# minh86/ModelCrowdNav

Hardware: AMD Instinct MI355X
Metric: env-steps/sec (whole node), 5-human CrowdSim x batched envs (higher is better)
Workload: dtype f64

## Files before the change

modelcrowdnav_amd/csrc/env_rollout_quad.hip:

```cpp
#include <hip/hip_runtime.h>
#include <stdint.h>
#include "../../include/mcn.h"
#include "quad_common.hpp"
#include "env_step_params.hpp"
#include "env_common.hpp"

namespace mcn {
void note_dispatch(const char *family);
void note_rollout_form(int form);

#ifdef MCN_DIAG
#define MCN_STAMP_SLOTS 64
#define MCN_STAMP_WAVES 8192
__device__ unsigned long long g_stamps[MCN_STAMP_WAVES * MCN_STAMP_SLOTS];
#define STAMP(slot)                                                                                              \
    do {                                                                                                         \
        const int w_ = blockIdx.x * (blockDim.x >> 6) + (threadIdx.x >> 6);                                      \
        if ((threadIdx.x & 63) == 0 && (slot) < MCN_STAMP_SLOTS && w_ < MCN_STAMP_WAVES)                         \
            g_stamps[w_ * MCN_STAMP_SLOTS + (slot)] = __builtin_amdgcn_s_memrealtime();                          \
    } while (0)
#define STAMP_WHERE()                                                                                            \
    do {                                                                                                         \
        const int w_ = blockIdx.x * (blockDim.x >> 6) + (threadIdx.x >> 6);                                      \
        if ((threadIdx.x & 63) == 0 && w_ < MCN_STAMP_WAVES)                                                     \
            g_stamps[w_ * MCN_STAMP_SLOTS + 38] =                                                                \
                (unsigned long long)__builtin_amdgcn_s_getreg((4) | (0 << 6) | (31 << 11)) |                     \
                ((unsigned long long)__builtin_amdgcn_s_getreg((20) | (0 << 6) | (31 << 11)) << 32);             \
    } while (0)
int read_counts(void *dst, size_t bytes, int reset)
{
    if (bytes > sizeof(g_diag_counts)) bytes = sizeof(g_diag_counts);
    const int rc = hipMemcpyFromSymbol(dst, HIP_SYMBOL(g_diag_counts), bytes) == hipSuccess ? (int)(bytes / 4) : -1;
    if (reset) {
        void *sym = nullptr;
        if (hipGetSymbolAddress(&sym, HIP_SYMBOL(g_diag_counts)) == hipSuccess) (void)hipMemset(sym, 0, sizeof(g_diag_counts));
    }
    return rc;
}
int read_stamps(void *dst, size_t bytes)
{
    if (bytes > sizeof(g_stamps)) bytes = sizeof(g_stamps);
    return hipMemcpyFromSymbol(dst, HIP_SYMBOL(g_stamps), bytes) == hipSuccess ? (int)(bytes / 8) : -1;
}
#else
#define STAMP(slot)
#define STAMP_WHERE()
#endif

__device__ __forceinline__ int bperm_i(int byte_addr, int v) { return __builtin_amdgcn_ds_bpermute(byte_addr, v); }
__device__ __forceinline__ float bperm_f(int byte_addr, float v)
{
    return __builtin_bit_cast(float, bperm_i(byte_addr, __builtin_bit_cast(int, v)));
}
__device__ __forceinline__ double bperm_d(int byte_addr, double v)
{
    const long long b = __builtin_bit_cast(long long, v);
    const int lo = bperm_i(byte_addr, (int)b), hi = bperm_i(byte_addr, (int)(b >> 32));
    return __builtin_bit_cast(double, ((long long)hi << 32) | (unsigned int)lo);
}

template <class V>
__device__ __forceinline__ V in_vgpr(V v)
{
    asm volatile("" : "+v"(v));
    return v;
}

typedef const __attribute__((address_space(4))) StepParams *KernargPtr;
__device__ __forceinline__ KernargPtr kernarg_here()
{
    KernargPtr q = (KernargPtr)__builtin_amdgcn_kernarg_segment_ptr();
    asm volatile("" : "+s"(q));
    return q;
}

template <int NT>
struct Wg4 {
    static_assert(NT == 5, "the four-wavefront form is built for 5 humans only");
    static constexpr int EW = 8;
    static constexpr int NQ = EW * NT;
};

template <int CTRL>
__device__ __forceinline__ int dpp_i(int v) { return __builtin_amdgcn_mov_dpp(v, CTRL, 0xf, 0xf, true); }
template <int CTRL>
__device__ __forceinline__ double dpp_d(double v)
{
    const long long b = __builtin_bit_cast(long long, v);
    const int lo = dpp_i<CTRL>((int)b), hi = dpp_i<CTRL>((int)(b >> 32));
    return __builtin_bit_cast(double, ((long long)hi << 32) | (unsigned int)lo);
}
constexpr int DPP_QUAD_XOR1 = 0xB1, DPP_QUAD_XOR2 = 0x4E, DPP_ROW_HALF_MIRROR = 0x141;

template <int NT, int VIS, bool UNI>
__device__ __forceinline__ void rollout_wg4(const StepParams &p, const int T)
{
    static_assert(VIS == 0, "the four-wavefront form is built for an invisible robot only");
    constexpr int EW = Wg4<NT>::EW, NQ = Wg4<NT>::NQ;
    __shared__ float4 s_opa[NQ], s_opb[NQ];
    __shared__ float2 s_res[NQ];
    __shared__ double2 s_hpos[NQ];
    __shared__ double s_hrad[NQ];
    STAMP(0);
    STAMP_WHERE();
#ifdef MCN_DIAG
    if (p.debug_noop) return;
#endif
    const int tid = threadIdx.x;
    const int role = __builtin_amdgcn_readfirstlane(tid >> 6);
    const unsigned nb_ = gridDim.x, xcd_ = blockIdx.x & 7u, idx_ = blockIdx.x >> 3;
    const unsigned qq_ = nb_ >> 3, rr__ = nb_ & 7u;
    const unsigned chunk_ = (xcd_ < rr__ ? xcd_ * (qq_ + 1) : rr__ * (qq_ + 1) + (xcd_ - rr__) * qq_) + idx_;
    const mcn_env_cfg &c = p.cfg;
    const mcn_rollout &ro = p.roll;

    if (role < 3) {
        const int lane = tid & 63, k = tid & 3, q = tid >> 2;
        const bool pop = q < NQ;
        const int ge = q / NT, h = q - ge * NT;
        const bool active = pop && (long)chunk_ * EW + ge < p.E;
        const int hi = pop ? q : 0;
        const bool cand_h = k < NT - 1;
        const int j = cand_h ? k + (k >= h ? 1 : 0) : h;
        const int ci = pop ? ge * NT + j : 0;
        const bool publish = pop && k == 0;
        const float inv_th = in_vgpr(1.0f / c.orca_time_horizon), inv_ts = in_vgpr(1.0f / (float)c.time_step);
        __syncthreads();
        STAMP(1);

        for (int t = 0; t < T; ++t) {
            const float4 A = s_opa[hi], B = s_opb[hi], o = s_opa[ci];
            const float orad = s_opb[ci].z;
            float rx, ry;
            quad_orca_core(c, lane, k, cand_h && active, A, B, o, orad, inv_th, inv_ts, rx, ry);
            if (publish) s_res[hi] = make_float2(rx, ry);
            if (t < 20) STAMP(40 + t);
            __syncthreads();
            __syncthreads();
            if (t < 37) STAMP(2 + t);
        }
    } else {
        static_assert(EW * 8 == 64, "eight lanes per env fill the wavefront");
        const double dt = in_vgpr(c.time_step);
        const bool do_reset = p.has_roll && ro.pool_hpos != nullptr;
        const int l = tid & 63;
        const int g = l >> 3, h = l & 7;
        const bool pop = h < NT;
        const int hs = g * NT + (pop ? h : 0);
        const long e = (long)chunk_ * EW + g;
        const bool active = pop && e < p.E;
        const long eb = e < p.E ? e : 0;
        const long a = eb * NT + (pop ? h : 0);
        const bool lead = active && h == 0;
        constexpr bool unicycle = UNI;
        const bool has_state = p.has_roll && ro.state != nullptr;
        const bool track = c.track_human_times && p.st.human_times != nullptr;

        double2 pos = reinterpret_cast<const double2 *>(p.st.hpos)[a];
        double2 vel = reinterpret_cast<const double2 *>(p.st.hvel)[a];
        double2 goal = reinterpret_cast<const double2 *>(p.st.hgoal)[a];
        double rad = p.st.hrad[a];
        double vpref = p.st.hvpref[a];
        double htime = p.st.human_times ? p.st.human_times[a] : 0.0;
        double hax = 0, hay = 0;
        double2 rpos = reinterpret_cast<const double2 *>(p.st.rpos)[eb];
        double2 rvel = reinterpret_cast<const double2 *>(p.st.rvel)[eb];
        double2 rgoal = reinterpret_cast<const double2 *>(p.st.rgoal)[eb];
        const double rrad = p.st.rrad[eb];
        double gtime = p.st.gtime[eb];
        double rtheta = p.st.rtheta ? p.st.rtheta[eb] : 0.0;
        mcn_roll_rec rs = {0, 0, 0, 0, 0, 0};
        if (has_state) rs = ro.state[eb];
        const double2 *act_ptr = reinterpret_cast<const double2 *>(p.actions) + eb;
        const long act_stride = in_vgpr((long)p.E);
        const double *disc_table = in_vgpr(ro.disc_table);
        const int disc_last = in_vgpr(ro.disc_len - 1);
        const bool has_theta = p.st.rtheta != nullptr;
        double2 act_next = *act_ptr;
        double o_rew = 0, o_dmin = 0;
        int o_dn = 0, o_inf = 0, o_hh = 0;
        const double k_timeout_at = in_vgpr(c.time_limit - 1);
        const double k_collision = in_vgpr(c.collision_penalty), k_success = in_vgpr(c.success_reward);
        const double k_discomfort = in_vgpr(c.discomfort_dist), k_factor = in_vgpr(c.discomfort_penalty_factor);
        const int k_stride = ro.case_stride, k_pool = ro.pool_size;
        const bool count_hh = c.count_hh != 0;
        {
            float4 A, B;
            quad_orca_operands(c, pos, vel, goal, rad, vpref, A, B);
            if (pop) { s_opa[hs] = A; s_opb[hs] = B; s_hpos[hs] = pos; s_hrad[hs] = rad; }
        }
        __syncthreads();
        STAMP(1);

        for (int t = 0; t < T; ++t) {
            const double2 act = act_next;
            act_ptr += act_stride;
            if (t + 1 < T) act_next = *act_ptr;
            double ep_disc = 0;
            if (has_state) ep_disc = disc_table[rs.ep_steps < disc_last ? rs.ep_steps : disc_last];

            double2 eff = act;
            if (unicycle) {
                eff.x = act.x * cos(act.y + rtheta);
                eff.y = act.x * sin(act.y + rtheta);
            }
            double cd;
            {
                const double px = pos.x - rpos.x, py = pos.y - rpos.y;
                const double vx = vel.x - eff.x, vy = vel.y - eff.y;
                cd = p2s_origin(px, py, px + vx * dt, py + vy * dt) - rad - rrad;
            }
            cd = pop ? cd : INFINITY;
            int hh = 0;
            {
                static_assert(NT / 2 == 2, "two pairs per lane");
                double s2[2], ra[2], rb[2];
                bool near_any = false;
                const bool counted = active & count_hh;
#pragma unroll
                for (int d = 1; d <= NT / 2; ++d) {
                    const int jj = h + d >= NT ? h + d - NT : h + d;
                    const int pi = g * NT + (pop ? jj : 0);
                    const double2 ppos = s_hpos[pi];
                    const double prad = s_hrad[pi];
                    ra[d - 1] = jj > h ? rad : prad; rb[d - 1] = jj > h ? prad : rad;
                    const double dx = pos.x - ppos.x, dy = pos.y - ppos.y;
                    s2[d - 1] = dx * dx + dy * dy;
                    const double reach = ra[d - 1] + rb[d - 1] + 1e-6;
                    near_any |= counted & (s2[d - 1] < reach * reach);
                }
                if (__any(near_any)) {
                    DIAG_COUNT(2);
#pragma unroll
                    for (int d = 0; d < NT / 2; ++d)
                        hh += (counted & ((sqrt(s2[d]) - ra[d] - rb[d]) < 0)) ? 1 : 0;
                }
            }
            double dmin = cd;
            int hh_sum = hh;
            dmin = fmin(dmin, dpp_d<DPP_QUAD_XOR1>(dmin));       hh_sum += dpp_i<DPP_QUAD_XOR1>(hh_sum);
            dmin = fmin(dmin, dpp_d<DPP_QUAD_XOR2>(dmin));       hh_sum += dpp_i<DPP_QUAD_XOR2>(hh_sum);
            dmin = fmin(dmin, dpp_d<DPP_ROW_HALF_MIRROR>(dmin)); hh_sum += dpp_i<DPP_ROW_HALF_MIRROR>(hh_sum);

            double endx, endy, new_theta = rtheta, nrvx, nrvy;
            if (unicycle) {
                const double th = rtheta + act.y;
                endx = rpos.x + cos(th) * act.x * dt;
                endy = rpos.y + sin(th) * act.x * dt;
                new_theta = pymod(rtheta + act.y, 2 * M_PI);
                nrvx = act.x * cos(new_theta); nrvy = act.x * sin(new_theta);
            } else {
                endx = rpos.x + act.x * dt; endy = rpos.y + act.y * dt;
                nrvx = act.x; nrvy = act.y;
            }
            bool reaching = false;
            {
                const double gx = endx - rgoal.x, gy = endy - rgoal.y, near = rrad + 1e-6;
                if (__any(gx * gx + gy * gy < near * near)) DIAG_COUNT(3);
                if (__any(gx * gx + gy * gy < near * near)) reaching = norm2(gx, gy) < rrad;
            }
            double rew; int inf, dn;
            if (gtime >= k_timeout_at)          { rew = 0; dn = 1; inf = MCN_INFO_TIMEOUT; }
            else if (dmin < 0)                  { rew = k_collision; dn = 1; inf = MCN_INFO_COLLISION; }
            else if (reaching)                  { rew = k_success; dn = 1; inf = MCN_INFO_REACHGOAL; }
            else if (dmin < k_discomfort)       { rew = (dmin - k_discomfort) * k_factor * dt; dn = 0; inf = MCN_INFO_DANGER; }
            else                                { rew = 0; dn = 0; inf = MCN_INFO_NOTHING; }
            o_rew = rew; o_dmin = dmin; o_dn = dn; o_inf = inf; o_hh = hh_sum;
            const double t_new = gtime + dt;

            const int case_g = rs.next_case;
            if (has_state) {
                bool danger = inf == MCN_INFO_DANGER;
                if (danger) {
                    const KernargPtr kp = kernarg_here();
                    const int lim = kp->roll.danger_episodes, sf = kp->roll.danger_short_from;
                    danger = lim <= 0 || rs.fin_count < lim - ((sf > 0 && e >= sf - 1) ? 1 : 0);
                }
                rs.danger_count += danger ? 1 : 0;
                rs.danger_dist_sum = danger ? rs.danger_dist_sum + dmin : rs.danger_dist_sum;
                const double ret = rs.ep_return + ep_disc * rew;
                if (lead && dn) {
                    const int kf = rs.fin_count;
                    const KernargPtr kp = kernarg_here();
                    const int fin_slots = kp->roll.fin_slots;
                    double *fin_return = kp->roll.fin_return, *fin_time = kp->roll.fin_time;
                    uint8_t *fin_info = kp->roll.fin_info;
                    const bool keep = (fin_slots == 1) || (kf < fin_slots);
                    const long rec = (long)(fin_slots == 1 ? 0 : kf) * kp->E + e;
                    if (keep && fin_return) fin_return[rec] = ret;
                    if (keep && fin_time)   fin_time[rec] = (inf == MCN_INFO_TIMEOUT) ? kp->cfg.time_limit : t_new;
                    if (keep && fin_info)   fin_info[rec] = (uint8_t)inf;
                }
                rs.fin_count += dn;
                rs.ep_return = dn ? 0.0 : ret;
                rs.ep_steps = dn ? 0 : rs.ep_steps + 1;
                if (do_reset) {
                    int nc = rs.next_case + k_stride;
                    nc = nc >= k_pool ? nc - k_pool : nc;
                    rs.next_case = dn ? nc : rs.next_case;
                }
            }

            if (do_reset && dn) {
                const KernargPtr kp = kernarg_here();
                const double k_theta0 = kp->roll.robot_theta0;
                rpos = make_double2(kp->roll.robot_start[0], kp->roll.robot_start[1]);
                rgoal = make_double2(kp->roll.robot_goal[0], kp->roll.robot_goal[1]);
                rvel = make_double2(0, 0);
                if (has_theta) rtheta = k_theta0;
                gtime = 0;
            } else {
                rpos = make_double2(endx, endy);
                rvel = make_double2(nrvx, nrvy);
                if (unicycle) rtheta = new_theta;
                gtime = t_new;
            }

            double2 npos = pos, nvel = vel, ngoal = goal;
            double nrad = rad, nvpref = vpref;
            if (do_reset && dn) {
                DIAG_COUNT(1);
                if (active) {
                    const long pa = (long)case_g * NT + h;
                    const KernargPtr kp = kernarg_here();
                    const double2 *pool_hvel = reinterpret_cast<const double2 *>(kp->roll.pool_hvel);
                    nvel = make_double2(0, 0);
                    if (pool_hvel) nvel = pool_hvel[pa];
                    npos = reinterpret_cast<const double2 *>(kp->roll.pool_hpos)[pa];
                    ngoal = reinterpret_cast<const double2 *>(kp->roll.pool_hgoal)[pa];
                    nrad = kp->roll.pool_hrad[pa];
                    nvpref = kp->roll.pool_hvpref[pa];
                }
            }

            if (t < 20) STAMP(40 + t);
            __syncthreads();
            {
                const float2 r = s_res[hs];
                hax = (double)r.x; hay = (double)r.y;
            }

            if (do_reset && dn) {
                pos = npos; vel = nvel; goal = ngoal; rad = nrad; vpref = nvpref;
                htime = 0;
            } else {
                pos = make_double2(pos.x + hax * dt, pos.y + hay * dt);
                vel = make_double2(hax, hay);
                if (track && htime == 0 && norm2(pos.x - goal.x, pos.y - goal.y) < rad) htime = t_new;
            }
            {
                float4 A, B;
                quad_orca_operands(c, pos, vel, goal, rad, vpref, A, B);
                if (pop) { s_opa[hs] = A; s_opb[hs] = B; s_hpos[hs] = pos; s_hrad[hs] = rad; }
            }
            __syncthreads();
            if (t < 37) STAMP(2 + t);
        }

        long a2 = a, e2 = e;
        asm volatile("" : "+v"(a2), "+v"(e2));
        const KernargPtr kp = kernarg_here();
        if (active) {
            reinterpret_cast<double2 *>(kp->st.hpos)[a2] = pos;
            reinterpret_cast<double2 *>(kp->st.hvel)[a2] = vel;
            if (do_reset) {
                reinterpret_cast<double2 *>(kp->st.hgoal)[a2] = goal;
                kp->st.hrad[a2] = rad;
                kp->st.hvpref[a2] = vpref;
            }
            double *human_times = kp->st.human_times, *human_act = kp->out.human_act;
            if (human_times) human_times[a2] = htime;
            if (human_act) reinterpret_cast<double2 *>(human_act)[a2] = make_double2(hax, hay);
        }
        if (lead) {
            reinterpret_cast<double2 *>(kp->st.rpos)[e2] = rpos;
            reinterpret_cast<double2 *>(kp->st.rvel)[e2] = rvel;
            if (do_reset) reinterpret_cast<double2 *>(kp->st.rgoal)[e2] = rgoal;
            double *rth = kp->st.rtheta;
            if (rth) rth[e2] = rtheta;
            kp->st.gtime[e2] = gtime;
            store_step_rec(kp->out.rec + e2, o_rew, o_dmin, o_dn, o_inf, o_hh);
            if (has_state) kp->roll.state[e2] = rs;
        }
    }
    STAMP(39);
}

template <int NT, int VIS, bool UNI>
__global__ __launch_bounds__(256, 2) void env_rollout_wg4_kernel(const StepParams p, const int T)
{
    rollout_wg4<NT, VIS, UNI>(p, T);
}

template <int NT, int VIS, bool UNI, bool SPLIT>
__global__ __launch_bounds__(SPLIT ? 128 : 64, SPLIT ? 3 : 1) void env_rollout_quad_kernel(const StepParams p, const int T)
{
    __shared__ double2 s_hpos[16], s_hvel[16], s_rpos[16], s_rvel[16];
    __shared__ double s_hrad[16];
    __shared__ int s_dn[16], s_case[16];
    STAMP(0);
    STAMP_WHERE();
#ifdef MCN_DIAG
    if (p.debug_noop) return;
#endif
    const int role = SPLIT ? (int)(threadIdx.x >> 6) : -1;
    const bool do_orca = role != 1, do_pair = role != 0;
    constexpr int NC = NT - 1 + VIS;
    constexpr int LPE = 4 * NT;
    constexpr int G = 64 / LPE;
    static_assert(NC >= 0 && NC <= 4, "quad kernel handles at most 4 ORCA neighbours");
    const int lane = threadIdx.x & 63;
    const int g = lane / LPE;
    const int r = lane - g * LPE;
    const int h = r >> 2, k = r & 3;
#ifndef MCN_QUAD_XCD
#define MCN_QUAD_XCD 1
#endif
    const unsigned nb_ = gridDim.x, xcd_ = blockIdx.x & 7u, idx_ = blockIdx.x >> 3;
    const unsigned qq_ = nb_ >> 3, rr__ = nb_ & 7u;
    const unsigned chunk_ = MCN_QUAD_XCD ? (xcd_ < rr__ ? xcd_ * (qq_ + 1) : rr__ * (qq_ + 1) + (xcd_ - rr__) * qq_) + idx_
                                         : blockIdx.x;
    const long e = (long)chunk_ * G + g;
    const bool active = (g < G) && (e < p.E);
    const long eb = active ? e : 0;
    const long a = eb * NT + h;
    const int gi = g < G ? g : 0;
    const int hi = g < G ? g * NT + h : 0;
    const mcn_env_cfg &c = p.cfg;
    const mcn_rollout &ro = p.roll;
    const double dt = in_vgpr(c.time_step);
    const bool lead = active && r == 0 && do_pair;
    const bool hlead = active && k == 0 && do_orca;
    constexpr bool unicycle = UNI;
    const bool has_state = p.has_roll && ro.state != nullptr;
    const bool do_reset = p.has_roll && ro.pool_hpos != nullptr;
    const bool track = c.track_human_times && p.st.human_times != nullptr;

    double2 pos = reinterpret_cast<const double2 *>(p.st.hpos)[a];
    double2 vel = reinterpret_cast<const double2 *>(p.st.hvel)[a];
    double2 goal = reinterpret_cast<const double2 *>(p.st.hgoal)[a];
    double rad = p.st.hrad[a];
    double vpref = p.st.hvpref[a];
    double htime = p.st.human_times ? p.st.human_times[a] : 0.0;
    double2 rpos = reinterpret_cast<const double2 *>(p.st.rpos)[eb];
    double2 rvel = reinterpret_cast<const double2 *>(p.st.rvel)[eb];
    double2 rgoal = reinterpret_cast<const double2 *>(p.st.rgoal)[eb];
    const double rrad = p.st.rrad[eb];
    double gtime = p.st.gtime[eb];
    double rtheta = p.st.rtheta ? p.st.rtheta[eb] : 0.0;
    mcn_roll_rec rs = {0, 0, 0, 0, 0, 0};
    if (has_state) rs = ro.state[eb];

    const bool cand_h = k < NT - 1;
    const bool cand_r = VIS && (k == NT - 1);
    const int j = cand_h ? k + (k >= h ? 1 : 0) : h;
    const int l0 = lane - r;
    const int src = ((l0 + 4 * j) & 63) << 2;

    const double2 *act_ptr = reinterpret_cast<const double2 *>(p.actions) + eb;
    const long act_stride = in_vgpr((long)p.E);
    const double *disc_table = in_vgpr(ro.disc_table);
    const int disc_last = in_vgpr(ro.disc_len - 1);
    const bool has_theta = p.st.rtheta != nullptr;
    double2 act_next = *act_ptr;
    double o_rew = 0, o_dmin = 0;
    int o_dn = 0, o_inf = 0, o_hh = 0;
    double hax = 0, hay = 0;
    const float inv_th = in_vgpr(1.0f / c.orca_time_horizon), inv_ts = in_vgpr(1.0f / (float)c.time_step);
    STAMP(1);

    for (int t = 0; t < T; ++t) {
        const double2 act = act_next;
        act_ptr += act_stride;
        if (do_pair && t + 1 < T) act_next = *act_ptr;
        double ep_disc = 0;
        if (do_pair && has_state) ep_disc = disc_table[rs.ep_steps < disc_last ? rs.ep_steps : disc_last];

        double2 cpos;
        cpos.x = bperm_d(src, pos.x);
        cpos.y = bperm_d(src, pos.y);
        double crd = bperm_d(src, rad);
        float cvx = bperm_f(src, (float)vel.x), cvy = bperm_f(src, (float)vel.y);
        if (cand_r) { cpos = rpos; crd = rrad; }

        int dn = 0, case_g = 0;
        double t_new = 0;

        if (do_orca) {
            if (cand_r) { cvx = (float)rvel.x; cvy = (float)rvel.y; }
            float rx, ry;
            quad_orca_velocity(c, lane, k, (cand_h || cand_r) && active, pos, vel, goal, rad, vpref,
                               make_float4((float)cpos.x, (float)cpos.y, cvx, cvy), crd, inv_th, inv_ts, rx, ry);
            hax = (double)rx; hay = (double)ry;
        }

        if (do_pair) {
            double2 eff = act;
            if (unicycle) {
                eff.x = act.x * cos(act.y + rtheta);
                eff.y = act.x * sin(act.y + rtheta);
            }
            double cd;
            {
                const double px = pos.x - rpos.x, py = pos.y - rpos.y;
                const double vx = vel.x - eff.x, vy = vel.y - eff.y;
                cd = p2s_origin(px, py, px + vx * dt, py + vy * dt) - rad - rrad;
            }
            int hh = 0;
            {
                const double dx = pos.x - cpos.x, dy = pos.y - cpos.y;
                const bool counted = active & (c.count_hh != 0) & cand_h & (j > h);
                const double s2 = dx * dx + dy * dy, reach = rad + crd + 1e-6;
                if (__any(counted & (s2 < reach * reach))) DIAG_COUNT(2);
                if (__any(counted & (s2 < reach * reach)))
                    hh = (counted & ((sqrt(s2) - rad - crd) < 0)) ? 1 : 0;
            }
            hh += __builtin_amdgcn_update_dpp(0, hh, 0xB1, 0xf, 0xf, false);
            hh += __builtin_amdgcn_update_dpp(0, hh, 0x4E, 0xf, 0xf, false);
            double dmin = INFINITY;
            int hh_sum = 0;
#pragma unroll
            for (int q = 0; q < NT; ++q) {
                const int s = (l0 + 4 * q) & 63;
                dmin = fmin(dmin, __shfl(cd, s));
                hh_sum += __shfl(hh, s);
            }

            double endx, endy, new_theta = rtheta, nrvx, nrvy;
            if (unicycle) {
                const double th = rtheta + act.y;
                endx = rpos.x + cos(th) * act.x * dt;
                endy = rpos.y + sin(th) * act.x * dt;
                new_theta = pymod(rtheta + act.y, 2 * M_PI);
                nrvx = act.x * cos(new_theta); nrvy = act.x * sin(new_theta);
            } else {
                endx = rpos.x + act.x * dt; endy = rpos.y + act.y * dt;
                nrvx = act.x; nrvy = act.y;
            }
            bool reaching = false;
            {
                const double gx = endx - rgoal.x, gy = endy - rgoal.y, near = rrad + 1e-6;
                if (__any(gx * gx + gy * gy < near * near)) DIAG_COUNT(3);
                if (__any(gx * gx + gy * gy < near * near)) reaching = norm2(gx, gy) < rrad;
            }
            const KernargPtr kc = kernarg_here();
            const double k_time_limit = kc->cfg.time_limit, k_timeout_at = k_time_limit - 1;
            const double k_collision = kc->cfg.collision_penalty, k_success = kc->cfg.success_reward;
            const double k_discomfort = kc->cfg.discomfort_dist, k_factor = kc->cfg.discomfort_penalty_factor;
            double rew; int inf;
            if (gtime >= k_timeout_at)          { rew = 0; dn = 1; inf = MCN_INFO_TIMEOUT; }
            else if (dmin < 0)                  { rew = k_collision; dn = 1; inf = MCN_INFO_COLLISION; }
            else if (reaching)                  { rew = k_success; dn = 1; inf = MCN_INFO_REACHGOAL; }
            else if (dmin < k_discomfort)       { rew = (dmin - k_discomfort) * k_factor * dt; dn = 0; inf = MCN_INFO_DANGER; }
            else                                { rew = 0; dn = 0; inf = MCN_INFO_NOTHING; }
            o_rew = rew; o_dmin = dmin; o_dn = dn; o_inf = inf; o_hh = hh_sum;
            t_new = gtime + dt;

            case_g = rs.next_case;
            if (has_state) {
                bool danger = inf == MCN_INFO_DANGER;
                if (danger) {
                    const KernargPtr kp = kernarg_here();
                    const int lim = kp->roll.danger_episodes, sf = kp->roll.danger_short_from;
                    danger = lim <= 0 || rs.fin_count < lim - ((sf > 0 && e >= sf - 1) ? 1 : 0);
                }
                rs.danger_count += danger ? 1 : 0;
                rs.danger_dist_sum = danger ? rs.danger_dist_sum + dmin : rs.danger_dist_sum;
                const double ret = rs.ep_return + ep_disc * rew;
                if (lead && dn) {
                    const int kf = rs.fin_count;
                    const KernargPtr kp = kernarg_here();
                    const int fin_slots = kp->roll.fin_slots;
                    double *fin_return = kp->roll.fin_return, *fin_time = kp->roll.fin_time;
                    uint8_t *fin_info = kp->roll.fin_info;
                    const bool keep = (fin_slots == 1) || (kf < fin_slots);
                    const long rec = (long)(fin_slots == 1 ? 0 : kf) * kp->E + e;
                    if (keep && fin_return) fin_return[rec] = ret;
                    if (keep && fin_time)   fin_time[rec] = (inf == MCN_INFO_TIMEOUT) ? k_time_limit : t_new;
                    if (keep && fin_info)   fin_info[rec] = (uint8_t)inf;
                }
                rs.fin_count += dn;
                rs.ep_return = dn ? 0.0 : ret;
                rs.ep_steps = dn ? 0 : rs.ep_steps + 1;
                if (do_reset) {
                    const int k_stride = kc->roll.case_stride, k_pool = kc->roll.pool_size;
                    int nc = rs.next_case + k_stride;
                    nc = nc >= k_pool ? nc - k_pool : nc;
                    rs.next_case = dn ? nc : rs.next_case;
                }
            }

            if (do_reset && dn) {
                const KernargPtr kp = kernarg_here();
                const double k_theta0 = kp->roll.robot_theta0;
                rpos = make_double2(kp->roll.robot_start[0], kp->roll.robot_start[1]);
                rgoal = make_double2(kp->roll.robot_goal[0], kp->roll.robot_goal[1]);
                rvel = make_double2(0, 0);
                if (has_theta) rtheta = k_theta0;
                gtime = 0;
            } else {
                rpos = make_double2(endx, endy);
                rvel = make_double2(nrvx, nrvy);
                if (unicycle) rtheta = new_theta;
                gtime = t_new;
            }
        }

        if (SPLIT) {
            if (lead) {
                s_dn[gi] = dn; s_case[gi] = case_g;
                if (VIS) { s_rpos[gi] = rpos; s_rvel[gi] = rvel; }
            }
            __syncthreads();
            if (role == 0) {
                dn = s_dn[gi]; case_g = s_case[gi];
                if (VIS) { rpos = s_rpos[gi]; rvel = s_rvel[gi]; }
            }
        }

        if (do_orca) {
            if (do_reset && dn) {
                DIAG_COUNT(1);
                if (active) {
                    const long pa = (long)case_g * NT + h;
                    const KernargPtr kp = kernarg_here();
                    const double2 *pool_hvel = reinterpret_cast<const double2 *>(kp->roll.pool_hvel);
                    pos = reinterpret_cast<const double2 *>(kp->roll.pool_hpos)[pa];
                    goal = reinterpret_cast<const double2 *>(kp->roll.pool_hgoal)[pa];
                    rad = kp->roll.pool_hrad[pa];
                    vpref = kp->roll.pool_hvpref[pa];
                    vel = pool_hvel ? pool_hvel[pa] : make_double2(0, 0);
                }
                htime = 0;
            } else {
                pos = make_double2(pos.x + hax * dt, pos.y + hay * dt);
                vel = make_double2(hax, hay);
                if (track && htime == 0 && norm2(pos.x - goal.x, pos.y - goal.y) < rad) htime = SPLIT ? gtime + dt : t_new;
            }
        }
        if (SPLIT) {
            if (role == 0) gtime = (do_reset && dn) ? 0.0 : gtime + dt;
            if (hlead) { s_hpos[hi] = pos; s_hvel[hi] = vel; s_hrad[hi] = rad; }
            __syncthreads();
            if (role == 1) { pos = s_hpos[hi]; vel = s_hvel[hi]; rad = s_hrad[hi]; }
        }
        if (t < 37) STAMP(2 + t);
    }

    {
        long a2 = a, e2 = e;
        asm volatile("" : "+v"(a2), "+v"(e2));
        const KernargPtr kp = kernarg_here();
        if (hlead) {
            reinterpret_cast<double2 *>(kp->st.hpos)[a2] = pos;
            reinterpret_cast<double2 *>(kp->st.hvel)[a2] = vel;
            if (do_reset) {
                reinterpret_cast<double2 *>(kp->st.hgoal)[a2] = goal;
                kp->st.hrad[a2] = rad;
                kp->st.hvpref[a2] = vpref;
            }
            double *human_times = kp->st.human_times, *human_act = kp->out.human_act;
            if (human_times) human_times[a2] = htime;
            if (human_act) reinterpret_cast<double2 *>(human_act)[a2] = make_double2(hax, hay);
        }
        if (lead) {
            reinterpret_cast<double2 *>(kp->st.rpos)[e2] = rpos;
            reinterpret_cast<double2 *>(kp->st.rvel)[e2] = rvel;
            if (do_reset) reinterpret_cast<double2 *>(kp->st.rgoal)[e2] = rgoal;
            double *rth = kp->st.rtheta;
            if (rth) rth[e2] = rtheta;
            kp->st.gtime[e2] = gtime;
            store_step_rec(kp->out.rec + e2, o_rew, o_dmin, o_dn, o_inf, o_hh);
            if (has_state) kp->roll.state[e2] = rs;
        }
    }
    STAMP(39);
}

template <int NT, int VIS, bool UNI>
static void launch_rollout_kin(const StepParams &p, int T, int blocks, hipStream_t stream)
{
    if constexpr (NT == 5 && VIS == 0) {
        if (p.quad_split == 2) {
            constexpr int EW = Wg4<NT>::EW;
            hipLaunchKernelGGL((env_rollout_wg4_kernel<NT, VIS, UNI>), dim3((p.E + EW - 1) / EW), dim3(256), 0, stream, p, T);
            note_rollout_form(2);
            return;
        }
    }
    if (p.quad_split)
        hipLaunchKernelGGL((env_rollout_quad_kernel<NT, VIS, UNI, true>), dim3(blocks), dim3(128), 0, stream, p, T);
    else
        hipLaunchKernelGGL((env_rollout_quad_kernel<NT, VIS, UNI, false>), dim3(blocks), dim3(64), 0, stream, p, T);
    note_rollout_form(p.quad_split ? 1 : 0);
}

template <int NT, int VIS>
static void launch_rollout_one(const StepParams &p, int T, hipStream_t stream)
{
    constexpr int G = 64 / (4 * NT);
    const int blocks = (p.E + G - 1) / G;
    if (p.cfg.robot_kinematics == MCN_KIN_UNICYCLE)
        launch_rollout_kin<NT, VIS, true>(p, T, blocks, stream);
    else
        launch_rollout_kin<NT, VIS, false>(p, T, blocks, stream);
}

bool launch_env_rollout_quad(const StepParams &p, int T, hipStream_t stream)
{
    if (p.cfg.human_policy != MCN_HUMANS_ORCA || p.cfg.orca_max_neighbors < 4 || !p.update) return false;
    const int vis = p.cfg.robot_visible ? 1 : 0;
    const int nc = p.N - 1 + vis;
    if (nc > 4 || p.N < 1) return false;
    switch (p.N * 2 + vis) {
        case 2:  launch_rollout_one<1, 0>(p, T, stream); break;
        case 3:  launch_rollout_one<1, 1>(p, T, stream); break;
        case 4:  launch_rollout_one<2, 0>(p, T, stream); break;
        case 5:  launch_rollout_one<2, 1>(p, T, stream); break;
        case 6:  launch_rollout_one<3, 0>(p, T, stream); break;
        case 7:  launch_rollout_one<3, 1>(p, T, stream); break;
        case 8:  launch_rollout_one<4, 0>(p, T, stream); break;
        case 9:  launch_rollout_one<4, 1>(p, T, stream); break;
        case 10: launch_rollout_one<5, 0>(p, T, stream); break;
        default: return false;
    }
    note_dispatch("env_rollout_quad_kernel");
    return true;
}

}
```

modelcrowdnav_amd/csrc/quad_common.hpp:

```cpp
#pragma once
#include <hip/hip_runtime.h>
#include "orca_device.hpp"
#include "orca_static.hpp"

namespace mcn {

#ifdef MCN_DIAG
static __device__ unsigned int g_diag_counts[8192 * 4];
#define DIAG_COUNT(which)                                                                                        \
    do {                                                                                                         \
        const int w_ = blockIdx.x * (blockDim.x >> 6) + (threadIdx.x >> 6);                                      \
        if (w_ < 8192 && (int)(threadIdx.x & 63) == __ffsll((unsigned long long)__ballot(1)) - 1)                \
            atomicAdd(&g_diag_counts[w_ * 4 + (which)], 1u);                                                     \
    } while (0)
#else
#define DIAG_COUNT(which)
#endif

template <int I>
__device__ __forceinline__ int qbi(int v) { return __builtin_amdgcn_mov_dpp(v, I * 0x55, 0xf, 0xf, false); }
template <int I>
__device__ __forceinline__ float qbf(float v) { return __builtin_bit_cast(float, qbi<I>(__builtin_bit_cast(int, v))); }
template <int I>
__device__ __forceinline__ double qbd(double v)
{
    const long long b = __builtin_bit_cast(long long, v);
    const int lo = qbi<I>((int)b), hi = qbi<I>((int)(b >> 32));
    return __builtin_bit_cast(double, ((long long)hi << 32) | (unsigned int)lo);
}
template <int I>
__device__ __forceinline__ float4 qb4(float4 v) { return make_float4(qbf<I>(v.x), qbf<I>(v.y), qbf<I>(v.z), qbf<I>(v.w)); }

__device__ __forceinline__ float4 sel4(const float4 (&L)[4], int i)
{
    const float4 a = i == 1 ? L[1] : L[0], b = i == 3 ? L[3] : L[2];
    return i >= 2 ? b : a;
}

template <bool DIR>
__device__ __forceinline__ bool lp1_rt(const float4 (&L)[4], const float4 &ln, int no, float radius, float optx, float opty,
                                       float &rx, float &ry)
{
    const float dp = dot2(ln.x, ln.y, ln.z, ln.w);
    const float disc = dp * dp + radius * radius - dot2(ln.x, ln.y, ln.x, ln.y);
    bool ok = !(disc < 0.0f);
    const float sq = sqrt_f32(disc, ok);
    float tl = -dp - sq;
    float tr = -dp + sq;
#pragma unroll
    for (int i = 0; i < 3; ++i) {
        const float4 li = L[i];
        const float den = det2(ln.z, ln.w, li.z, li.w);
        const float num = det2(li.z, li.w, ln.x - li.x, ln.y - li.y);
        const float t = num / den;
        const bool live = i < no;
        const bool par = fabsf(den) <= kRvoEps;
        const bool cut = live & !par;
        const float ntr = fminf(tr, t), ntl = fmaxf(tl, t);
        tr = (cut & (den >= 0.0f)) ? ntr : tr;
        tl = (cut & !(den >= 0.0f)) ? ntl : tl;
        ok = ok & !(live & ((par ? 0.0f : tl) > (par ? num : tr)));
    }
    float t;
    if (DIR) {
        t = (dot2(optx, opty, ln.z, ln.w) > 0.0f) ? tr : tl;
    } else {
        t = dot2(ln.z, ln.w, optx - ln.x, opty - ln.y);
        if (t < tl) t = tl; else if (t > tr) t = tr;
    }
    rx = ln.x + t * ln.z;
    ry = ln.y + t * ln.w;
    return ok;
}

__device__ __forceinline__ bool lp3_candidate_quad(const float4 &li, const float4 &lj, int i, int k, float radius, float &rx,
                                                   float &ry)
{
    const float dt = det2(li.z, li.w, lj.z, lj.w);
    const bool par = fabsf(dt) <= kRvoEps;
    const bool same = dot2(li.z, li.w, lj.z, lj.w) > 0.0f;
    const bool keptb = (k < i) & !(par & same);
    const unsigned long long m_kept = lanes(k < i) & ~(lanes(par) & lanes(same));
    const float sc = det2(lj.z, lj.w, li.x - lj.x, li.y - lj.y) / dt;
    const float ddx = lj.z - li.z, ddy = lj.w - li.w;
    const float inv = keptb ? rcp_sqrt_f32(dot2(ddx, ddy, ddx, ddy), m_kept) : 0.0f;
    const float4 q = make_float4(par ? 0.5f * (li.x + lj.x) : li.x + sc * li.z,
                                 par ? 0.5f * (li.y + lj.y) : li.y + sc * li.w, ddx * inv, ddy * inv);
    const float4 P0 = qb4<0>(q), P1 = qb4<1>(q), P2 = qb4<2>(q);
    const float ox = -li.w, oy = li.z;

    const float dp = dot2(q.x, q.y, q.z, q.w);
    const float disc = dp * dp + radius * radius - dot2(q.x, q.y, q.x, q.y);
    bool ok = !(disc < 0.0f);
    const float sq = sqrt_f32(disc, lanes(!(disc < 0.0f)) & m_kept);
    float tl = -dp - sq;
    float tr = -dp + sq;
#pragma unroll
    for (int j = 0; j < 2; ++j) {
        const float4 pj = j == 0 ? P0 : P1;
        const bool live = j < k;
        const float den = det2(q.z, q.w, pj.z, pj.w);
        const float num = det2(pj.z, pj.w, q.x - pj.x, q.y - pj.y);
        const float t = num / den;
        const bool parj = fabsf(den) <= kRvoEps;
        const bool cut = live & !parj;
        const float ntr = fminf(tr, t), ntl = fmaxf(tl, t);
        tr = (cut & (den >= 0.0f)) ? ntr : tr;
        tl = (cut & !(den >= 0.0f)) ? ntl : tl;
        ok = ok & !(live & ((parj ? 0.0f : tl) > (parj ? num : tr)));
    }
    const float tt = (dot2(ox, oy, q.z, q.w) > 0.0f) ? tr : tl;
    const float cx = q.x + tt * q.z, cy = q.y + tt * q.w;
    const int fcode = ok ? 4 : k;

    rx = radius * ox; ry = radius * oy;
    int fail = 3;
#define MCN_LP3_INNER_TAKE(I, PI)                                                              \
    {                                                                                          \
        const int code_i = qbi<I>(fcode); const float cx_i = qbf<I>(cx), cy_i = qbf<I>(cy);    \
        const bool out = det2(PI.z, PI.w, PI.x - rx, PI.y - ry) > 0.0f;                         \
        fail = ((fail > I) & out) ? min(fail, code_i) : fail;                                   \
        const bool take = (fail > I) & out;                                                     \
        rx = take ? cx_i : rx; ry = take ? cy_i : ry;                                           \
    }
    MCN_LP3_INNER_TAKE(0, P0) MCN_LP3_INNER_TAKE(1, P1) MCN_LP3_INNER_TAKE(2, P2)
#undef MCN_LP3_INNER_TAKE
    return fail == 3;
}

__device__ __forceinline__ void quad_orca_operands(const mcn_env_cfg &c, double2 pos, double2 vel, double2 goal, double rad,
                                                   double vpref, float4 &A, float4 &B)
{
    const float fpx = (float)pos.x, fpy = (float)pos.y, fvx = (float)vel.x, fvy = (float)vel.y;
    const float frad = (float)(rad + 0.01 + c.orca_safety_space);
    const float ms = (float)vpref;
    const float prefx = (float)(goal.x - pos.x), prefy = (float)(goal.y - pos.y);
    A = make_float4(fpx, fpy, fvx, fvy);
    B = make_float4(prefx, prefy, frad, ms);
}

__device__ __forceinline__ void quad_orca_core(const mcn_env_cfg &c, int lane, int k, bool cand_valid, float4 A, float4 B,
                                               float4 o, float orad, float inv_th, float inv_ts, float &rx, float &ry);

__device__ __forceinline__ void quad_orca_velocity(const mcn_env_cfg &c, int lane, int k, bool cand_valid,
                                                   double2 pos, double2 vel, double2 goal, double rad, double vpref,
                                                   float4 o, double crd, float inv_th, float inv_ts, float &rx, float &ry)
{
    float4 A, B;
    quad_orca_operands(c, pos, vel, goal, rad, vpref, A, B);
    const float orad = (float)(crd + 0.01 + c.orca_safety_space);
    quad_orca_core(c, lane, k, cand_valid, A, B, o, orad, inv_th, inv_ts, rx, ry);
}

__device__ __forceinline__ void quad_orca_core(const mcn_env_cfg &c, int lane, int k, bool cand_valid, float4 A, float4 B,
                                               float4 o, float orad, float inv_th, float inv_ts, float &rx, float &ry)
{
    const float fpx = A.x, fpy = A.y, fvx = A.z, fvy = A.w;
    const float prefx = B.x, prefy = B.y, frad = B.z, ms = B.w;
    const float range_sq = c.orca_neighbor_dist * c.orca_neighbor_dist;
    const float ddx = fpx - o.x, ddy = fpy - o.y;
    const float d = dot2(ddx, ddy, ddx, ddy);
    const bool in = cand_valid && (d < range_sq);
    const int key = in ? __builtin_bit_cast(int, d) : 0x7f800000;
    const int kd0 = qbi<0>(key) - key, kd1 = qbi<1>(key) - key, kd2 = qbi<2>(key) - key, kd3 = qbi<3>(key) - key;
    const int rank = (kd0 < (0 < k ? 1 : 0)) + (kd1 < (1 < k ? 1 : 0)) + (kd2 < (2 < k ? 1 : 0)) + (kd3 < 0);
    const int nin = __builtin_popcount((unsigned)(__builtin_amdgcn_ballot_w64(in) >> (lane & ~3)) & 0xfu);
    const int nl = nin < c.orca_max_neighbors ? nin : c.orca_max_neighbors;
    const float4 mine = orca_line_select(fpx, fpy, fvx, fvy, frad, o, orad, inv_th, inv_ts, in);
    const int dst = ((lane & ~3) | rank) << 2;
    float4 srt;
    srt.x = __builtin_bit_cast(float, __builtin_amdgcn_ds_permute(dst, __builtin_bit_cast(int, mine.x)));
    srt.y = __builtin_bit_cast(float, __builtin_amdgcn_ds_permute(dst, __builtin_bit_cast(int, mine.y)));
    srt.z = __builtin_bit_cast(float, __builtin_amdgcn_ds_permute(dst, __builtin_bit_cast(int, mine.z)));
    srt.w = __builtin_bit_cast(float, __builtin_amdgcn_ds_permute(dst, __builtin_bit_cast(int, mine.w)));
    {
        const float pp = dot2(prefx, prefy, prefx, prefy);
        const bool clip = pp > ms * ms;
        const float inv = rcp_sqrt_f32(pp, clip);
        rx = clip ? ms * (prefx * inv) : prefx;
        ry = clip ? ms * (prefy * inv) : prefy;
    }
    const float4 L[4] = {qb4<0>(srt), qb4<1>(srt), qb4<2>(srt), qb4<3>(srt)};

    float cx, cy;
    const int fcode = lp1_rt<false>(L, srt, k, ms, prefx, prefy, cx, cy) ? 4 : k;
    int fail = nl;
#define MCN_LP2_TAKE(I)                                                                        \
    {                                                                                          \
        const int code_i = qbi<I>(fcode); const float cx_i = qbf<I>(cx), cy_i = qbf<I>(cy);    \
        const bool out = det2(L[I].z, L[I].w, L[I].x - rx, L[I].y - ry) > 0.0f;                 \
        fail = ((fail > I) & out) ? min(fail, code_i) : fail;                                   \
        const bool take = (fail > I) & out;                                                     \
        rx = take ? cx_i : rx; ry = take ? cy_i : ry;                                           \
    }
    MCN_LP2_TAKE(0) MCN_LP2_TAKE(1) MCN_LP2_TAKE(2) MCN_LP2_TAKE(3)
#undef MCN_LP2_TAKE
    if (fail < nl) {
        DIAG_COUNT(0);
        float dist = 0.0f;
        int i = fail;
        for (;;) {
            const unsigned long long over = lanes((unsigned)(k - i) < (unsigned)(nl - i)) &
                                            lanes(det2(srt.z, srt.w, srt.x - rx, srt.y - ry) > dist);
            const unsigned m = (unsigned)(over >> (lane & ~3)) & 0xfu;
            if (m == 0) break;
            const int nxt = __builtin_ctz(m);
            const float4 ln = sel4(L, nxt);
            float cx3, cy3;
            const bool ok3 = lp3_candidate_quad(ln, srt, nxt, k, ms, cx3, cy3);
            rx = ok3 ? cx3 : rx; ry = ok3 ? cy3 : ry;
            dist = det2(ln.z, ln.w, ln.x - rx, ln.y - ry);
            i = nxt + 1;
        }
    }
}

}
```

Baseline: 1.892 billion.

## Double-buffer shared state so ORCA waves integrate positions, dropping one barrier per step

The ORCA worker wavefronts now keep each human's state in registers and integrate positions themselves. They publish the updated position and velocity into double-buffered shared arrays. The step-function wave sends fresh operands only when an episode resets, signalled by a per-env flag. This removes one of the two __syncthreads per step and the redundant operand recomputation in the step wave. In exchange it uses more LDS and duplicates the double-precision integration across lanes, which risks subtle consistency bugs around resets.

```diff
diff --git a/modelcrowdnav_amd/csrc/env_rollout_quad.hip b/modelcrowdnav_amd/csrc/env_rollout_quad.hip
--- a/modelcrowdnav_amd/csrc/env_rollout_quad.hip
+++ b/modelcrowdnav_amd/csrc/env_rollout_quad.hip
@@ -97,9 +97,9 @@
 {
     static_assert(VIS == 0, "the four-wavefront form is built for an invisible robot only");
     constexpr int EW = Wg4<NT>::EW, NQ = Wg4<NT>::NQ;
-    __shared__ float4 s_opa[NQ], s_opb[NQ];
-    __shared__ float2 s_res[NQ];
-    __shared__ double2 s_hpos[NQ];
+    __shared__ float4 s_pa[2][NQ], s_ra[2][NQ], s_rb[2][NQ];
+    __shared__ double2 s_pos[2][2 * NQ], s_rgoal[2][NQ];
+    __shared__ int s_flag[2][EW];
     __shared__ double s_hrad[NQ];
     STAMP(0);
     STAMP_WHERE();
@@ -120,23 +120,52 @@
         const int ge = q / NT, h = q - ge * NT;
         const bool active = pop && (long)chunk_ * EW + ge < p.E;
         const int hi = pop ? q : 0;
+        const int gi = pop ? ge : 0;
         const bool cand_h = k < NT - 1;
         const int j = cand_h ? k + (k >= h ? 1 : 0) : h;
         const int ci = pop ? ge * NT + j : 0;
         const bool publish = pop && k == 0;
         const float inv_th = in_vgpr(1.0f / c.orca_time_horizon), inv_ts = in_vgpr(1.0f / (float)c.time_step);
+        const double dt = in_vgpr(c.time_step);
+        double2 pos = make_double2(0, 0), goal = make_double2(0, 0);
+        float fpx = 0, fpy = 0, fvx = 0, fvy = 0, prefx = 0, prefy = 0, frad = 0, ms = 0;
+        float4 o = make_float4(0, 0, 0, 0);
+        float orad = 0;
+        auto fetch = [&](const int par) {
+            o = s_pa[par][ci];
+            const int flag = s_flag[par][gi];
+            if (__any(flag != 0)) {
+                const float4 ra = s_ra[par][hi], rb = s_rb[par][hi], rc = s_ra[par][ci];
+                const double2 rp = s_pos[par][NQ + hi], rg = s_rgoal[par][hi];
+                const float ro_ = s_rb[par][ci].z;
+                if (flag != 0) {
+                    pos = rp; goal = rg;
+                    fpx = ra.x; fpy = ra.y; fvx = ra.z; fvy = ra.w;
+                    prefx = rb.x; prefy = rb.y; frad = rb.z; ms = rb.w;
+                    o = rc; orad = ro_;
+                }
+            }
+        };
         __syncthreads();
+        fetch(0);
         STAMP(1);
 
         for (int t = 0; t < T; ++t) {
-            const float4 A = s_opa[hi], B = s_opb[hi], o = s_opa[ci];
-            const float orad = s_opb[ci].z;
+            const int nb = (t + 1) & 1;
             float rx, ry;
-            quad_orca_core(c, lane, k, cand_h && active, A, B, o, orad, inv_th, inv_ts, rx, ry);
-            if (publish) s_res[hi] = make_float2(rx, ry);
+            quad_orca_core(c, lane, k, cand_h && active, make_float4(fpx, fpy, fvx, fvy), make_float4(prefx, prefy, frad, ms),
+                           o, orad, inv_th, inv_ts, rx, ry);
+            pos = make_double2(pos.x + (double)rx * dt, pos.y + (double)ry * dt);
+            fvx = rx; fvy = ry;
+            fpx = (float)pos.x; fpy = (float)pos.y;
+            if (publish) { s_pa[nb][hi] = make_float4(fpx, fpy, fvx, fvy); s_pos[nb][hi] = pos; }
+            prefx = (float)(goal.x - pos.x); prefy = (float)(goal.y - pos.y);
             if (t < 20) STAMP(40 + t);
             __syncthreads();
-            __syncthreads();
+            fetch(nb);
+#ifdef MCN_DIAG
+            asm volatile("s_waitcnt lgkmcnt(0)" ::: "memory");
+#endif
             if (t < 37) STAMP(2 + t);
         }
     } else {
@@ -187,12 +216,15 @@
         {
             float4 A, B;
             quad_orca_operands(c, pos, vel, goal, rad, vpref, A, B);
-            if (pop) { s_opa[hs] = A; s_opb[hs] = B; s_hpos[hs] = pos; s_hrad[hs] = rad; }
-        }
+            if (pop) { s_ra[0][hs] = A; s_rb[0][hs] = B; s_pos[0][NQ + hs] = pos; s_rgoal[0][hs] = goal; s_hrad[hs] = rad; }
+            if (h == 0) s_flag[0][g] = 1;
+        }
+        bool rst = true;
         __syncthreads();
         STAMP(1);
 
         for (int t = 0; t < T; ++t) {
+            const int cur = t & 1, nb = cur ^ 1;
             const double2 act = act_next;
             act_ptr += act_stride;
             if (t + 1 < T) act_next = *act_ptr;
@@ -221,7 +253,7 @@
                 for (int d = 1; d <= NT / 2; ++d) {
                     const int jj = h + d >= NT ? h + d - NT : h + d;
                     const int pi = g * NT + (pop ? jj : 0);
-                    const double2 ppos = s_hpos[pi];
+                    const double2 ppos = s_pos[cur][(rst ? NQ : 0) + pi];
                     const double prad = s_hrad[pi];
                     ra[d - 1] = jj > h ? rad : prad; rb[d - 1] = jj > h ? prad : rad;
                     const double dx = pos.x - ppos.x, dy = pos.y - ppos.y;
@@ -316,9 +348,10 @@
                 gtime = t_new;
             }
 
+            const bool rst_now = do_reset && dn;
             double2 npos = pos, nvel = vel, ngoal = goal;
             double nrad = rad, nvpref = vpref;
-            if (do_reset && dn) {
+            if (rst_now) {
                 DIAG_COUNT(1);
                 if (active) {
                     const long pa = (long)case_g * NT + h;
@@ -333,27 +366,30 @@
                 }
             }
 
+            if (rst_now) {
+                float4 A, B;
+                quad_orca_operands(c, npos, nvel, ngoal, nrad, nvpref, A, B);
+                if (pop) { s_ra[nb][hs] = A; s_rb[nb][hs] = B; s_pos[nb][NQ + hs] = npos; s_rgoal[nb][hs] = ngoal; s_hrad[hs] = nrad; }
+            }
+            if (h == 0) s_flag[nb][g] = rst_now ? 1 : 0;
+
             if (t < 20) STAMP(40 + t);
             __syncthreads();
+
             {
-                const float2 r = s_res[hs];
-                hax = (double)r.x; hay = (double)r.y;
-            }
-
-            if (do_reset && dn) {
-                pos = npos; vel = nvel; goal = ngoal; rad = nrad; vpref = nvpref;
-                htime = 0;
-            } else {
-                pos = make_double2(pos.x + hax * dt, pos.y + hay * dt);
-                vel = make_double2(hax, hay);
-                if (track && htime == 0 && norm2(pos.x - goal.x, pos.y - goal.y) < rad) htime = t_new;
-            }
-            {
-                float4 A, B;
-                quad_orca_operands(c, pos, vel, goal, rad, vpref, A, B);
-                if (pop) { s_opa[hs] = A; s_opb[hs] = B; s_hpos[hs] = pos; s_hrad[hs] = rad; }
-            }
-            __syncthreads();
+                const float4 na = s_pa[nb][hs];
+                const double2 np_ = s_pos[nb][hs];
+                hax = (double)na.z; hay = (double)na.w;
+                if (rst_now) {
+                    pos = npos; vel = nvel; goal = ngoal; rad = nrad; vpref = nvpref;
+                    htime = 0;
+                } else {
+                    pos = np_;
+                    vel = make_double2(hax, hay);
+                    if (track && htime == 0 && norm2(pos.x - goal.x, pos.y - goal.y) < rad) htime = t_new;
+                }
+                rst = rst_now;
+            }
             if (t < 37) STAMP(2 + t);
         }
 
```

Result: faster. 1.929 billion (median of 6 runs) (+1.9%).

## Repack ORCA shared operands and reuse velocity result buffer with double buffering

Applied to the files above, without the earlier changes.

Splits the shared ORCA operand arrays into a position/preference pack, a rad/vpref array that changes only on reset, and a double-buffered velocity array. The solver wavefronts now read the previous step's velocity result directly as the operand velocity. The update wavefront therefore rewrites only the position pack each step and rewrites radius and preferred speed only for reset envs. The aim is less per-step LDS write traffic and conversion work on the update wavefront, which sits on the critical path between the two barriers. The parity indexing and split writes add complexity and the risk of subtle ordering bugs across the two barriers.

```diff
diff --git a/modelcrowdnav_amd/csrc/env_rollout_quad.hip b/modelcrowdnav_amd/csrc/env_rollout_quad.hip
--- a/modelcrowdnav_amd/csrc/env_rollout_quad.hip
+++ b/modelcrowdnav_amd/csrc/env_rollout_quad.hip
@@ -97,8 +97,8 @@
 {
     static_assert(VIS == 0, "the four-wavefront form is built for an invisible robot only");
     constexpr int EW = Wg4<NT>::EW, NQ = Wg4<NT>::NQ;
-    __shared__ float4 s_opa[NQ], s_opb[NQ];
-    __shared__ float2 s_res[NQ];
+    __shared__ float4 s_pack[NQ];
+    __shared__ float2 s_res[2 * NQ], s_inv[NQ];
     __shared__ double2 s_hpos[NQ];
     __shared__ double s_hrad[NQ];
     STAMP(0);
@@ -125,15 +125,23 @@
         const int ci = pop ? ge * NT + j : 0;
         const bool publish = pop && k == 0;
         const float inv_th = in_vgpr(1.0f / c.orca_time_horizon), inv_ts = in_vgpr(1.0f / (float)c.time_step);
+        int rd_h = hi + NQ, rd_c = ci + NQ;
         __syncthreads();
         STAMP(1);
 
         for (int t = 0; t < T; ++t) {
-            const float4 A = s_opa[hi], B = s_opb[hi], o = s_opa[ci];
-            const float orad = s_opb[ci].z;
+            float4 P = s_pack[hi];
+            float2 cp = *reinterpret_cast<const float2 *>(s_pack + ci);
+            float2 v = s_res[rd_h], cv = s_res[rd_c];
+            float2 fm = s_inv[hi];
+            float orad = s_inv[ci].x;
+            asm volatile("" : "+v"(P.x), "+v"(P.y), "+v"(P.z), "+v"(P.w), "+v"(cp.x), "+v"(cp.y), "+v"(v.x), "+v"(v.y),
+                              "+v"(cv.x), "+v"(cv.y), "+v"(fm.x), "+v"(fm.y), "+v"(orad));
             float rx, ry;
-            quad_orca_core(c, lane, k, cand_h && active, A, B, o, orad, inv_th, inv_ts, rx, ry);
-            if (publish) s_res[hi] = make_float2(rx, ry);
+            quad_orca_core(c, lane, k, cand_h && active, make_float4(P.x, P.y, v.x, v.y), make_float4(P.z, P.w, fm.x, fm.y),
+                           make_float4(cp.x, cp.y, cv.x, cv.y), orad, inv_th, inv_ts, rx, ry);
+            if (publish) s_res[(t & 1) * NQ + hi] = make_float2(rx, ry);
+            rd_h = in_vgpr(hi + (t & 1) * NQ); rd_c = in_vgpr(ci + (t & 1) * NQ);
             if (t < 20) STAMP(40 + t);
             __syncthreads();
             __syncthreads();
@@ -187,7 +195,11 @@
         {
             float4 A, B;
             quad_orca_operands(c, pos, vel, goal, rad, vpref, A, B);
-            if (pop) { s_opa[hs] = A; s_opb[hs] = B; s_hpos[hs] = pos; s_hrad[hs] = rad; }
+            if (pop) {
+                s_pack[hs] = make_float4(A.x, A.y, B.x, B.y); s_res[NQ + hs] = make_float2(A.z, A.w);
+                s_inv[hs] = make_float2(B.z, B.w);
+                s_hpos[hs] = pos; s_hrad[hs] = rad;
+            }
         }
         __syncthreads();
         STAMP(1);
@@ -316,45 +328,56 @@
                 gtime = t_new;
             }
 
-            double2 npos = pos, nvel = vel, ngoal = goal;
-            double nrad = rad, nvpref = vpref;
-            if (do_reset && dn) {
+            const bool restart = do_reset && dn;
+            float4 n_pack = make_float4(0, 0, 0, 0);
+            float2 n_fvel = make_float2(0, 0), n_inv = make_float2(0, 0);
+            if (restart) {
                 DIAG_COUNT(1);
                 if (active) {
                     const long pa = (long)case_g * NT + h;
                     const KernargPtr kp = kernarg_here();
                     const double2 *pool_hvel = reinterpret_cast<const double2 *>(kp->roll.pool_hvel);
-                    nvel = make_double2(0, 0);
-                    if (pool_hvel) nvel = pool_hvel[pa];
-                    npos = reinterpret_cast<const double2 *>(kp->roll.pool_hpos)[pa];
-                    ngoal = reinterpret_cast<const double2 *>(kp->roll.pool_hgoal)[pa];
-                    nrad = kp->roll.pool_hrad[pa];
-                    nvpref = kp->roll.pool_hvpref[pa];
-                }
-            }
+                    vel = make_double2(0, 0);
+                    if (pool_hvel) vel = pool_hvel[pa];
+                    pos = reinterpret_cast<const double2 *>(kp->roll.pool_hpos)[pa];
+                    goal = reinterpret_cast<const double2 *>(kp->roll.pool_hgoal)[pa];
+                    rad = kp->roll.pool_hrad[pa];
+                    vpref = kp->roll.pool_hvpref[pa];
+                }
+                htime = 0;
+                float4 A, B;
+                quad_orca_operands(c, pos, vel, goal, rad, vpref, A, B);
+                n_pack = make_float4(in_vgpr(A.x), in_vgpr(A.y), in_vgpr(B.x), in_vgpr(B.y));
+                n_fvel = make_float2(in_vgpr(A.z), in_vgpr(A.w));
+                n_inv = make_float2(in_vgpr(B.z), in_vgpr(B.w));
+            }
+            const bool any_restart = __any(restart);
 
             if (t < 20) STAMP(40 + t);
             __syncthreads();
+            float2 *vel_io = s_res + (t & 1) * NQ;
             {
-                const float2 r = s_res[hs];
+                const float2 r = vel_io[hs];
                 hax = (double)r.x; hay = (double)r.y;
             }
-
-            if (do_reset && dn) {
-                pos = npos; vel = nvel; goal = ngoal; rad = nrad; vpref = nvpref;
-                htime = 0;
-            } else {
+            if (!restart) {
                 pos = make_double2(pos.x + hax * dt, pos.y + hay * dt);
+                if (pop) s_pack[hs] = quad_orca_position_pack(pos, goal);
+            }
+            if (any_restart) {
+                if (pop && restart) { s_pack[hs] = n_pack; vel_io[hs] = n_fvel; s_inv[hs] = n_inv; }
+            }
+            __syncthreads();
+            if (t < 37) STAMP(2 + t);
+
+            if (pop) s_hpos[hs] = pos;
+            if (!restart) {
                 vel = make_double2(hax, hay);
                 if (track && htime == 0 && norm2(pos.x - goal.x, pos.y - goal.y) < rad) htime = t_new;
             }
-            {
-                float4 A, B;
-                quad_orca_operands(c, pos, vel, goal, rad, vpref, A, B);
-                if (pop) { s_opa[hs] = A; s_opb[hs] = B; s_hpos[hs] = pos; s_hrad[hs] = rad; }
-            }
-            __syncthreads();
-            if (t < 37) STAMP(2 + t);
+            if (any_restart) {
+                if (pop && restart) s_hrad[hs] = rad;
+            }
         }
 
         long a2 = a, e2 = e;
diff --git a/modelcrowdnav_amd/csrc/quad_common.hpp b/modelcrowdnav_amd/csrc/quad_common.hpp
--- a/modelcrowdnav_amd/csrc/quad_common.hpp
+++ b/modelcrowdnav_amd/csrc/quad_common.hpp
@@ -137,6 +137,11 @@
     const float prefx = (float)(goal.x - pos.x), prefy = (float)(goal.y - pos.y);
     A = make_float4(fpx, fpy, fvx, fvy);
     B = make_float4(prefx, prefy, frad, ms);
+}
+
+__device__ __forceinline__ float4 quad_orca_position_pack(double2 pos, double2 goal)
+{
+    return make_float4((float)pos.x, (float)pos.y, (float)(goal.x - pos.x), (float)(goal.y - pos.y));
 }
 
 __device__ __forceinline__ void quad_orca_core(const mcn_env_cfg &c, int lane, int k, bool cand_valid, float4 A, float4 B,
```

New measurement: 1.885 billion before, 1.925 billion after (median of 6 runs). +2.1%, better.
